# Plachtaa/FAcodec

Hardware: NVIDIA H100
Metric: audio_seconds_per_second (higher is better)
Workload: dtype f32 I/O and accumulation; every product is a 3-MMA split of fp32 operands: fp16 hi + 2^11-scaled fp16 lo (22 mantissa bits, register-promoted accumulation) upstream of the VQ, bf16 hi + bf16 lo (16 bits) downstream

## Files before the change

### facodec_b200/_lib.py

```python
import ctypes
import os

from . import build as _build

_c = ctypes
_LIB = None


class FacError(RuntimeError):
    pass


def lib_path():
    return _build.LIB


def load():
    global _LIB
    if _LIB is not None:
        return _LIB
    path = lib_path()
    if not os.path.exists(path):
        raise FacError(f"{path} not found: build it with `python -m facodec_b200.build` "
                       "(needs nvcc; there is no CPU fallback)")
# ... 37 lines not shown
        "fac_vc_stream_convert": ([vp, i32, i64p, i64p, i32, i32, fp, vp], i32),
        "fac_vc_stream_finish": ([vp, i32, fp, vp], i32),
        "fac_vc_stream_end": ([vp, i32], i32),
        "fac_spectral_loss": ([vp, fp, fp, i32, i32, i32, i32, _c.POINTER(_c.c_int), _c.POINTER(_c.c_int), fp, fp,
                               _c.c_float, _c.c_float, _c.c_float, _c.c_float, fp, vp], i32),
        "fac_l1_loss": ([vp, fp, fp, _c.c_longlong, fp, vp], i32),
        "fac_spectral_loss_grad": ([vp, fp, fp, i32, i32, i32, i32, _c.POINTER(_c.c_int), _c.POINTER(_c.c_int), fp, fp,
                                    _c.c_float, _c.c_float, _c.c_float, _c.c_float, fp, fp, fp, vp], i32),
        "fac_l1_loss_grad": ([vp, fp, fp, _c.c_longlong, fp, fp, fp, vp], i32),
        "fac_add3": ([vp, fp, fp, fp, _c.c_longlong, fp, vp], i32),
        "fac_reconstruction_loss": ([vp, fp, fp, i32, i32, fp, fp, vp], i32),
        "fac_rvq_forward": ([vp, i32, fp, i32, i32, i32, fp, i64p, fp, vp], i32),
        "fac_alias_free_act": ([vp, fp, i32, i32, i32, i32, fp, fp, fp, vp], i32),
        "fac_debug_conv": ([vp, fp, fp, fp] + [i32] * 10 + [fp, fp, i32, fp, fp, i32, vp], i32),
        "fac_debug_conv_tc": ([vp, fp, fp, fp] + [i32] * 10 + [fp, fp, i32, fp, fp, i32, i32, vp], i32),
        "fac_debug_resunit": ([vp, fp, fp, fp, fp, fp, fp, fp, i32, i32, i32, i32, i32, fp, vp], i32),
        "fac_debug_tc_phase_clocks": ([vp, _c.POINTER(_c.c_longlong)], i32),
        "fac_debug_tc_producer_clocks": ([vp, _c.POINTER(_c.c_longlong)], i32),
        "fac_debug_tc_trace": ([vp, _c.POINTER(_c.c_longlong)], i32),
        "fac_debug_lstm_pack": ([fp, i32, i32, fp, _c.c_longlong, _c.POINTER(_c.c_int)], _c.c_longlong),
        "fac_debug_convtr_pack": ([fp, i32, i32, i32, i32, fp, _c.c_longlong], _c.c_longlong),
        "fac_debug_pad_map": ([i32, i32, i32, i32, _c.POINTER(_c.c_int), i32], i32),
        "fac_debug_tc_plan": ([i32] * 8 + [_c.POINTER(_c.c_int)], i32),
        "fac_debug_tc_pack": ([fp, i32, i32, i32, i32, i32, fp, _c.c_longlong], _c.c_longlong),
        "fac_debug_lstm_phase_clocks": ([vp, _c.POINTER(_c.c_longlong)], i32),
        "fac_set_option": ([vp, _c.c_char_p, i32], i32),
        "fac_debug_slstm": ([vp, fp, _c.POINTER(vp), i32, i32, i32, i32, _c.POINTER(_c.c_int), i32, fp, vp], i32),
        "fac_debug_fa_quantize": ([vp, fp, fp, _c.POINTER(vp), fp, i32, i32, i32, i32, i32, fp, fp, fp, fp, i64p, i64p, i64p,
                                   fp, fp, vp], i32),
        "fac_debug_attention": ([vp, fp, fp, fp, fp, i32, i32, i32, _c.c_void_p, i32, vp], i32),
        "fac_debug_tap": ([vp, _c.c_char_p, fp, _c.c_size_t], i32),
        "fac_profile_enable": ([vp, i32], i32),
        "fac_profile_reset": ([vp], i32),
        "fac_profile_get": ([vp, _c.c_char_p, _c.POINTER(_c.c_double), _c.POINTER(_c.c_double),
                             _c.POINTER(_c.c_double), _c.POINTER(_c.c_longlong)], i32),
        "fac_profile_dump": ([vp, _c.c_char_p, _c.c_size_t], _c.c_size_t),
        "fac_workspace_bytes": ([vp], _c.c_size_t),
        "fac_last_launch_count": ([vp], i32),
    }
    for name, (args, res) in sigs.items():
        fn = getattr(L, name)
        fn.argtypes = args
        fn.restype = res
    _LIB = L
    return L


EXPORTED = ["fac_abi_version", "fac_create", "fac_destroy", "fac_last_error", "fac_load_tensor", "fac_finalize",
            "fac_encode", "fac_encode_frames", "fac_quantize", "fac_decode", "fac_codec_forward",
            "fac_codec_forward_host", "fac_codec_encode", "fac_dequantize", "fac_codes_decode", "fac_redecode", "fac_redecoder_decode", "fac_voice_convert", "fac_dataset_mel", "fac_reconstruction_loss", "fac_spectral_loss", "fac_l1_loss", "fac_spectral_loss_grad", "fac_l1_loss_grad", "fac_head_begin", "fac_head_tensor", "fac_head_finalize", "fac_head_forward", "fac_add3", "fac_stream_begin", "fac_stream_encode", "fac_stream_decode", "fac_stream_decode_codes", "fac_stream_encode_codes", "fac_stream_finish_codes", "fac_stream_end", "fac_vc_stream_lookahead", "fac_vc_stream_begin", "fac_vc_stream_convert", "fac_vc_stream_finish", "fac_vc_stream_end", "fac_rvq_create", "fac_rvq_destroy", "fac_rvq_forward", "fac_alias_free_act",
            "fac_debug_conv", "fac_debug_conv_tc", "fac_debug_resunit", "fac_debug_tc_phase_clocks", "fac_debug_tc_producer_clocks", "fac_debug_tc_trace", "fac_debug_lstm_pack", "fac_debug_convtr_pack", "fac_debug_pad_map", "fac_debug_tc_plan", "fac_debug_tc_pack", "fac_debug_lstm_phase_clocks", "fac_set_option", "fac_debug_slstm", "fac_debug_fa_quantize", "fac_debug_attention", "fac_debug_tap", "fac_profile_enable", "fac_profile_reset", "fac_profile_get", "fac_profile_dump",
            "fac_workspace_bytes", "fac_last_launch_count"]


def check(handle, rc, what):
    if rc < 0:
        msg = load().fac_last_error(handle)
        raise FacError(f"{what} failed (status {rc}): {msg.decode() if msg else ''}")
    return rc
```

### facodec_b200/csrc/conv_tc.cu

```cuda
#include <cuda_bf16.h>
#include <cuda_fp16.h>

#include <cstring>
#include <mutex>

#include "common.cuh"
#include "conv_tc_common.cuh"
#include "kernels.h"

namespace fac {

namespace {

using namespace tc;

enum Prec { P_TF32 = 0, P_BF16 = 1, P_F16S = 2, P_F16X2 = 3, P_NONE = -1 };

template <int P> struct PrecT {
    static constexpr int KG = P == P_TF32 ? 4 : 2;
    static constexpr int planes = P == P_F16S ? 1 : 2;
    static constexpr int ksteps = P == P_TF32 ? 2 : 1;
    static constexpr int kind = P == P_TF32 ? WG_TF32 : (P == P_BF16 ? WG_BF16 : WG_F16);
};

// ... 32 lines not shown
            const int row = tl.row0 + 16 * tl.warp + (tl.lane >> 2) + 8 * h;
            const int col = tl.col0 + 8 * j + 2 * (tl.lane & 3);
            f(row, col, acc[4 * j + 2 * h], acc[4 * j + 2 * h + 1]);
        }
    }
}

template <bool FAST>
__device__ __forceinline__ float act_out(int act, float v, float al, float ia) {
    if (act == ACT_SNAKE) return FAST ? fmaf(ia, sin2_mufu(al * v), v) : snake_fast(v, al, ia);
    if (act == ACT_TANH) return tanhf(v);
    if (act == ACT_MISH) return mish_f(v);
    return v;
}

template <int P1, int P2, bool PROMO, int NI, int MINB = 1, bool TT = false>
__global__ void __launch_bounds__(kThreads, MINB) conv_tc_kernel(TcConvParams p) {
    constexpr bool FUSED = P2 != P_NONE;
    static_assert(!TT || (NI == 64 && !FUSED), "transposed tiles: <= 64 channels x 64 time steps per warpgroup");
    static_assert(NI % 16 == 0 && NI <= (PROMO || MINB == 2 ? 64 : (P1 == P_F16S ? 256 : 128)),
                  "accumulator registers: <= 64 / 128 columns (256 in the one-pass fp16 class at one CTA per SM)");
    constexpr bool F16X2 = P1 == P_F16X2;
    constexpr bool DEC = P1 == P_BF16 || P1 == P_F16S;
    using T1 = PrecT<P1>;
    extern __shared__ __align__(1024) uint8_t smem[];
    uint64_t* full = reinterpret_cast<uint64_t*>(smem);

    const int tid = threadIdx.x, wg = tid >> 7;
    const int BM = 64 * p.MT;
    const int N = p.N, NW = p.MT == 2 ? N : N / 2;
    Tile tl;
    tl.row0 = p.MT == 2 ? 64 * wg : 0;
    tl.col0 = p.MT == 2 ? 0 : wg * NW;
    tl.nw = NW;
    tl.warp = (tid >> 5) & 3;
    tl.lane = tid & 31;
    const int t0 = blockIdx.x * BM, ntile = blockIdx.y, b = blockIdx.z;
    const int Kr = p.Kr, dil = p.dil, Rpad = p.Rpad, nchunk = p.nchunk, S = p.stagesB;
    const int R = BM + (Kr - 1) * dil;
    const uint32_t a_plane = (uint32_t)T1::KG * Rpad * 16, a_bytes = a_plane * T1::planes;
    uint8_t* abuf = smem + kSmemHdr;
    float4* master = reinterpret_cast<float4*>(abuf + 2 * (size_t)a_bytes);
    uint8_t* wbuf = abuf + 2 * (size_t)a_bytes + master_bytes(PROMO, nchunk, p.promote_every, NI);
    uint8_t* a2buf = wbuf + (size_t)S * p.b_slot;
    const uint32_t w_unit1 = (uint32_t)Kr * T1::planes * T1::KG * N * 16;
    const uint32_t w_unit2 = FUSED ? (uint32_t)prec_planes(P2) * prec_kg(P2) * N * 16 : 0;
    const int units = nchunk + (FUSED ? p.nchunk2 : 0);

    if (tid == 0) {
        for (int i = 0; i < S; ++i) mbar_init(&full[i], 1);
        fence_mbar_init();
    }
    __syncthreads();
    auto issue_w = [&](int u) {
        uint64_t* bar = &full[u % S];
        uint8_t* dst = wbuf + (size_t)(u % S) * p.b_slot;
        const uint8_t* src;
        uint32_t bytes;
        if (u < nchunk) { src = reinterpret_cast<const uint8_t*>(p.wblob) + ((size_t)ntile * nchunk + u) * w_unit1; bytes = w_unit1; }
        else { src = reinterpret_cast<const uint8_t*>(p.wblob2) + (size_t)(u - nchunk) * w_unit2; bytes = w_unit2; }
        mbar_arrive_expect_tx(bar, bytes);
        bulk_g2s(dst, src, bytes, bar);
    };
    if (tid == 0)
        for (int u = 0; u < S - 1 && u < units; ++u) issue_w(u);

    const PadMap pm = PadMap::make(p.Tin, p.pad_left_s, p.pad_right_s, p.reflect);
    const float* __restrict__ xb = p.x + (size_t)b * p.x_bstride;
    auto produce = [&](int c) {
        uint8_t* ahi = abuf + (size_t)(c & 1) * a_bytes;
        if constexpr (P1 == P_TF32) produce_chunk<kThreads, false>(p, pm, xb, c, t0, R, Rpad, ahi, ahi + a_plane, tid);
        else if constexpr (P1 == P_BF16) produce_chunk<kThreads, true>(p, pm, xb, c, t0, R, Rpad, ahi, ahi + a_plane, tid);
        else if constexpr (P1 == P_F16S) produce_chunk<kThreads, true, 4, false, false, true>(p, pm, xb, c, t0, R, Rpad, ahi, ahi, tid);
        else produce_chunk<kThreads, false, 4, false, true>(p, pm, xb, c, t0, R, Rpad, ahi, ahi + a_plane, tid);
        fence_proxy_async();
    };
    produce(0);

    float acc[NI / 2];
    float crs[F16X2 ? NI / 2 : 1];
    zero_acc<NI>(acc);
    if constexpr (F16X2) zero_acc<NI>(crs);
    const uint32_t a_lbo = (uint32_t)Rpad * 16, b_lbo = (uint32_t)N * 16;
    const uint32_t abase = smem_u32(abuf), wbase = smem_u32(wbuf), a2base = smem_u32(a2buf);
    const int BM2 = BM;

    auto promote = [&](bool first, bool last) {
        if constexpr (PROMO) {
#pragma unroll
// ... 11 lines not shown
                acc[4 * q + 0] = last ? m.x : 0.f;
                acc[4 * q + 1] = last ? m.y : 0.f;
                acc[4 * q + 2] = last ? m.z : 0.f;
                acc[4 * q + 3] = last ? m.w : 0.f;
            }
        }
    };

#pragma unroll 1
    for (int u = 0; u < units; ++u) {
        __syncthreads();
        if (tid == 0 && u + S - 1 < units) issue_w(u + S - 1);
        mbar_wait(&full[u % S], (uint32_t)(u / S) & 1u);
        const uint32_t wslot = wbase + (uint32_t)(u % S) * p.b_slot;
        wg_fence();
        if (u < nchunk) {
            const uint32_t a0 = abase + (uint32_t)(u & 1) * a_bytes + (uint32_t)tl.row0 * 16;
            const uint32_t b0 = wslot + (uint32_t)tl.col0 * 16;
#pragma unroll 1
            for (int tap = 0; tap < Kr; ++tap) {
                const uint32_t ahi = a0 + (uint32_t)(tap * dil) * 16, alo = ahi + a_plane;
                const uint32_t bhi = b0 + (uint32_t)tap * T1::planes * T1::KG * b_lbo, blo = bhi + T1::KG * b_lbo;
                if constexpr (TT) {
                    mma_pass<P1, NI>(acc, bhi, b_lbo, ahi, a_lbo);
                    mma_pass<P1, NI>(crs, bhi, b_lbo, alo, a_lbo);
                    mma_pass<P1, NI>(crs, blo, b_lbo, ahi, a_lbo);
                } else if constexpr (P1 == P_F16S) {
                    mma_pass<P1, NI>(acc, ahi, a_lbo, bhi, b_lbo);
                } else if constexpr (F16X2) {
                    mma_pass<P1, NI>(acc, ahi, a_lbo, bhi, b_lbo);
                    mma_pass<P1, NI>(crs, ahi, a_lbo, blo, b_lbo);
                    mma_pass<P1, NI>(crs, alo, a_lbo, bhi, b_lbo);
                } else {
                    mma_pass<P1, NI>(acc, ahi, a_lbo, bhi, b_lbo);
                    mma_pass<P1, NI>(acc, ahi, a_lbo, blo, b_lbo);
                    mma_pass<P1, NI>(acc, alo, a_lbo, bhi, b_lbo);
                }
            }
            wg_commit();
            if (u + 1 < nchunk) produce(u + 1);
            wg_wait_all();
            if (PROMO && ((u + 1) % p.promote_every == 0 || u + 1 == nchunk)) promote(u < p.promote_every, u + 1 == nchunk);
            if constexpr (FUSED) {
                if (u + 1 == nchunk) {
                    constexpr int KG2 = prec_kg(P2 < 0 ? 0 : P2);
                    const uint32_t a2_plane = (uint32_t)(p.nchunk2 * KG2) * BM2 * 16;
                    for_each_pair<NI, 32>(tl, acc, [&](int row, int col, float v0, float v1) {
                        const float2 bi = __ldg(reinterpret_cast<const float2*>(p.bias + col));
                        const float2 al = __ldg(reinterpret_cast<const float2*>(p.out_alpha + col));
                        const float2 ia = __ldg(reinterpret_cast<const float2*>(p.out_inv_alpha + col));
                        v0 = act_out<DEC>(ACT_SNAKE, v0 + bi.x, al.x, ia.x);
                        v1 = act_out<DEC>(ACT_SNAKE, v1 + bi.y, al.y, ia.y);
                        if constexpr (P2 == P_BF16) {
                            __nv_bfloat162 h = __floats2bfloat162_rn(v0, v1);
                            float2 hf = __bfloat1622float2(h);
                            __nv_bfloat162 l = __floats2bfloat162_rn(v0 - hf.x, v1 - hf.y);
                            const uint32_t off = ((uint32_t)(col >> 3) * BM2 + row) * 16 + (col & 7) * 2;
                            *reinterpret_cast<__nv_bfloat162*>(a2buf + off) = h;
                            *reinterpret_cast<__nv_bfloat162*>(a2buf + a2_plane + off) = l;
                        } else {
                            const float h0 = to_tf32(v0), h1 = to_tf32(v1);
                            const uint32_t off = ((uint32_t)(col >> 2) * BM2 + row) * 16 + (col & 3) * 4;
                            *reinterpret_cast<float2*>(a2buf + off) = make_float2(h0, h1);
                            *reinterpret_cast<float2*>(a2buf + a2_plane + off) = make_float2(to_tf32(v0 - h0), to_tf32(v1 - h1));
                        }
                    });
                    fence_proxy_async();
                    zero_acc<NI>(acc);
                }
            }
        } else if constexpr (FUSED) {
            constexpr int P2x = P2 < 0 ? 0 : P2;
            constexpr int KG2 = prec_kg(P2x);
            const int c2 = u - nchunk;
            const uint32_t a2_plane = (uint32_t)(p.nchunk2 * KG2) * BM2 * 16, a2_lbo = (uint32_t)BM2 * 16;
            const uint32_t ahi = a2base + ((uint32_t)(c2 * KG2) * BM2 + tl.row0) * 16, alo = ahi + a2_plane;
            const uint32_t bhi = wslot + (uint32_t)tl.col0 * 16, blo = bhi + KG2 * b_lbo;
            mma_pass<P2x, NI>(acc, ahi, a2_lbo, bhi, b_lbo);
            mma_pass<P2x, NI>(acc, ahi, a2_lbo, blo, b_lbo);
            mma_pass<P2x, NI>(acc, alo, a2_lbo, bhi, b_lbo);
            wg_commit();
            wg_wait_all();
        }
    }

    const float* __restrict__ bias = FUSED ? p.bias2 : p.bias;
    const int act = FUSED ? ACT_NONE : p.out_act;
    float* __restrict__ yb = p.y + (size_t)b * p.y_bstride + (size_t)ntile * N;
    const float* __restrict__ rb = p.res ? p.res + (size_t)b * p.y_bstride + (size_t)ntile * N : nullptr;
// ... 59 lines not shown
    p.nchunk2 = p.fused ? p.Cout / kChunk : 0;
    p.promote_every = p.promoted ? (p.f16x2 ? (48 / p.Kr < 1 ? 1 : 48 / p.Kr) : (8 / p.Kr < 1 ? 1 : 8 / p.Kr)) : 1;
    const int nw_max = p.promoted ? 64 : 128;
    constexpr size_t kAReserve = 40 * 1024;
    int N = 0;
    for (int cand = p.fused ? p.Cout : 256; cand >= 16 && N == 0; cand -= 16) {
        const bool rows_split = cand <= nw_max, cols_split = (cand / 2) % 16 == 0 && cand / 2 <= nw_max;
        if (p.Cout % cand || !(rows_split || cols_split)) continue;
        size_t slot = (size_t)p.Kr * prec_planes(P1) * prec_kg(P1) * cand * 16, a2 = 0;
        if (P2 != P_NONE) a2 = (size_t)prec_planes(P2) * p.nchunk2 * prec_kg(P2) * 64 * 16;
        if (kSmemHdr + kAReserve + slot + a2 <= kSmemCap) N = cand;
        else if (p.fused) return false;
    }
    if (N == 0) return false;
    struct Layout { int Rpad; size_t slot, total; };
    auto layout = [&](int S, int MT) {
        const int NW = MT == 2 ? N : N / 2, BM = 64 * MT;
        Layout l;
        l.Rpad = BM + (p.Kr - 1) * p.dil;
        while (l.Rpad % 8 != 2) ++l.Rpad;
        const size_t a_bytes = (size_t)prec_planes(P1) * prec_kg(P1) * l.Rpad * 16;
        l.slot = (size_t)p.Kr * prec_planes(P1) * prec_kg(P1) * N * 16;
        size_t a2 = 0;
        if (P2 != P_NONE) {
            const size_t slot2 = (size_t)prec_planes(P2) * prec_kg(P2) * N * 16;
            if (slot2 > l.slot) l.slot = slot2;
            a2 = (size_t)prec_planes(P2) * p.nchunk2 * prec_kg(P2) * BM * 16;
        }
        const size_t master = master_bytes(p.promoted, p.nchunk, p.promote_every, p.tt ? 64 : NW);
        l.total = kSmemHdr + 2 * a_bytes + master + S * l.slot + a2 + (p.tt ? 64 * 16 : 0);
        return l;
    };
    const bool want2 = p.promoted ? !p.tt : (p.occ2_maxn > 0 && N <= p.occ2_maxn);
    for (int two = want2 ? 1 : 0; two >= 0; --two) {
        const size_t cap = two ? kSmemCap2 : kSmemCap;
        const int nwl = two ? 64 : nw_max;
        for (int S = 2; S >= 1; --S)
            for (int MT = 2; MT >= 1; --MT) {
                const int NW = MT == 2 ? N : N / 2;
                const bool wide = !two && P1 == P_F16S && NW == f16s_wide_nw(p.fused);
                if ((NW > nwl && !wide) || NW % 16) continue;
                if (wide && layout(2, 1).total <= kSmemCap2) continue;
                const Layout l = layout(S, MT);
                if (l.total > cap) continue;
                p.N = N; p.MT = MT; p.Rpad = l.Rpad; p.R2pad = 64 * MT; p.stagesB = S; p.b_slot = (int)l.slot;
                p.smem_bytes = l.total;
                p.occ2 = two;
                return true;
            }
    }
    return false;
}

size_t tc_blob_floats(const TcConvParams& p) {
    if (p.g1f16) return (size_t)(p.Cout / p.N) * p.nchunk * p.Kr * 2 * p.N * 4;
    return (size_t)(p.Cout / p.N) * p.nchunk * p.Kr * 2 * ((p.bf16 || p.f16x2) ? 2 : 4) * p.N * 4;
}

static inline uint16_t bf16_rn_host(float f) {
    uint32_t u;
// ... 149 lines not shown
```

### facodec_b200/csrc/conv_tc_common.cuh

```cuda
#pragma once
#include <cuda_bf16.h>
#include <cuda_fp16.h>

#include "common.cuh"
#include "kernels.h"

namespace fac {

namespace tc {

constexpr int kThreads = 256;
constexpr int kChunk = 16;
constexpr int kSmemHdr = 128;

__device__ __forceinline__ uint32_t smem_u32(const void* p) { return (uint32_t)__cvta_generic_to_shared(p); }

__device__ __forceinline__ void mbar_init(uint64_t* bar, uint32_t count) {
    asm volatile("mbarrier.init.shared::cta.b64 [%0], %1;" ::"r"(smem_u32(bar)), "r"(count));
}
__device__ __forceinline__ void mbar_arrive(uint64_t* bar) {
    asm volatile("mbarrier.arrive.shared::cta.b64 _, [%0];" ::"r"(smem_u32(bar)) : "memory");
}
__device__ __forceinline__ void mbar_arrive_expect_tx(uint64_t* bar, uint32_t bytes) {
    asm volatile("mbarrier.arrive.expect_tx.shared::cta.b64 _, [%0], %1;" ::"r"(smem_u32(bar)), "r"(bytes) : "memory");
// ... 194 lines not shown
    uint2 hv, lv;
    hv.x = *reinterpret_cast<uint32_t*>(&h01); hv.y = *reinterpret_cast<uint32_t*>(&h23);
    lv.x = *reinterpret_cast<uint32_t*>(&l01); lv.y = *reinterpret_cast<uint32_t*>(&l23);
    *reinterpret_cast<uint2*>(ahi + off) = hv;
    *reinterpret_cast<uint2*>(alo + off) = lv;
}

__device__ __forceinline__ void store_f16_single(float4 x4, int pc, int row, int Rpad, uint8_t* ahi) {
    __half2 h01 = __floats2half2_rn(x4.x, x4.y), h23 = __floats2half2_rn(x4.z, x4.w);
    const size_t off = ((size_t)(pc >> 1) * Rpad + row) * 16 + (size_t)(pc & 1) * 8;
    uint2 hv;
    hv.x = *reinterpret_cast<uint32_t*>(&h01); hv.y = *reinterpret_cast<uint32_t*>(&h23);
    *reinterpret_cast<uint2*>(ahi + off) = hv;
}

template <int NT, bool BF16, int BATCH = 4, bool INL = false, bool F16 = false, bool SINGLE = false>
__device__ __forceinline__ void produce_chunk(const TcConvParams& p, const PadMap& pm, const float* __restrict__ xb,
                                              int c, int t0, int R, int Rpad, uint8_t* ahi, uint8_t* alo, int ptid) {
    const int pc = ptid & 3;
    const int j = c * kChunk + pc * 4;
    const int soff = j / p.Cin, ci = j - soff * p.Cin;
    const bool has_alpha = p.in_alpha != nullptr;
    float4 al = make_float4(0.f, 0.f, 0.f, 0.f), ia = al;
    if (has_alpha) {
        al = __ldg(reinterpret_cast<const float4*>(p.in_alpha + ci));
        ia = __ldg(reinterpret_cast<const float4*>(p.in_inv_alpha + ci));
    }
    constexpr int RSTEP = NT / 4;
    const int row_limit = p.Tout + (p.Kr - 1) * p.dil;
    const int vrow0 = t0 - p.PLr;
    const float* __restrict__ xcol = xb + ci;
#pragma unroll 1
    for (int r = ptid >> 2; r < R; r += RSTEP * BATCH) {
        float4 v[BATCH];
#pragma unroll
        for (int u = 0; u < BATCH; ++u) {
            const int rr = r + u * RSTEP;
            v[u] = make_float4(0.f, 0.f, 0.f, 0.f);
            const int vrow = vrow0 + rr;
            if (rr < R && vrow < row_limit) {
                const int src = pm.src(vrow * p.vf + soff);
                if (src >= 0) v[u] = __ldg(reinterpret_cast<const float4*>(xcol + (size_t)src * p.ldx));
            }
        }
#pragma unroll
        for (int u = 0; u < BATCH; ++u) {
            const int rr = r + u * RSTEP;
            if (rr < R) {
// ... 14 lines not shown
```

### facodec_b200/csrc/engine.cu

```cuda
#include <cmath>
#include <cstdio>
#include <cstdlib>
#include <cstring>
#include <map>
#include <string>
#include <vector>

#include "../../include/facodec_b200.h"
#include "../../include/facodec_b200_debug.h"
#include "common.cuh"
#include "kernels.h"

using namespace fac;

namespace {

constexpr int HOP = 300;
constexpr int LATENT = 1024;
constexpr int N_FFT = 2048;
constexpr int WIN = 1200;
constexpr int N_BINS = 1025;
constexpr int SPEC_LD = 2052;
constexpr int SPEC_TC_LD = 2176;
constexpr int N_MELS = 80;
// ... 2713 lines not shown
    if (std::string(name) == "fuse_resunit") { h->fuse_res = value < 0 ? 0 : (value > 2 ? 2 : value); return FAC_OK; }
    if (std::string(name) == "encoder_f16x2") { h->enc_f16 = value != 0; return FAC_OK; }
    if (std::string(name) == "encoder_tt") { h->enc_tt = value != 0; return FAC_OK; }
    if (std::string(name) == "tc_occ2_maxn") { h->tc_occ2 = value < 0 ? 0 : value; return FAC_OK; }
    if (std::string(name) == "decoder_conv7_fp16") { h->dec_c7_f16 = value != 0; return FAC_OK; }
    if (std::string(name) == "overlap_front") { h->overlap_front = value != 0; return FAC_OK; }
    if (std::string(name) == "lstm_v2") { h->lstm_v2 = value != 0; return FAC_OK; }
    if (std::string(name) == "decoder_lstm_fp16") { h->dec_lstm_fp16 = value != 0; return FAC_OK; }
    if (std::string(name) == "attention_stream") { h->attn_stream = value != 0; return FAC_OK; }
    if (std::string(name) == "decoder_bf16") { h->dec_bf16 = value != 0; return FAC_OK; }
    if (std::string(name) == "tensor_cores") { h->use_tc = value < 0 ? 0 : (value > 2 ? 2 : value); return FAC_OK; }
    h->err = std::string("unknown option ") + name;
    return FAC_ERR_INVALID;
}

int fac_debug_conv_tc(fac_handle* h, const float* x, const float* w_host, const float* bias_host, int B, int Tin, int Cin,
                      int Cout, int K, int dil, int stride, int pad_left, int pad_right, int reflect,
                      const float* in_alpha_host, const float* out_alpha_host, int act, const float* res, float* y,
                      int Tout, int promoted, void* stream) {
    if (!h || !x || !w_host || !y) return FAC_ERR_INVALID;
    cudaSetDevice(h->device);
    cudaStream_t st = (cudaStream_t)stream;
    TcConvParams tp;
    tp.Cin = Cin; tp.Cout = Cout; tp.promoted = (promoted == 1 || promoted == 3 || promoted == 4) ? 1 : 0;
    tp.bf16 = (promoted == 2 || promoted == 5) ? 1 : 0;
    tp.f16x2 = (promoted == 3 || promoted == 4) ? 1 : 0;
    tp.tt = promoted == 4 ? 1 : 0;
    tp.g1f16 = promoted == 5 ? 1 : 0;
    tp.occ2_maxn = h->tc_occ2;
    tp.Tout = Tout;
    if (stride == 1) { tp.vf = 1; tp.Kr = K; tp.dil = dil; }
    else if (K == 2 * stride && dil == 1) { tp.vf = stride; tp.Kr = 2; tp.dil = 1; }
    else { h->err = "fac_debug_conv_tc: unsupported stride/kernel"; return FAC_ERR_UNSUPPORTED; }
    if (promoted < 0 || promoted > 5 || !tc_conv_plan(tp)) { h->err = "fac_debug_conv_tc: layer not eligible for the tensor-core path"; return FAC_ERR_UNSUPPORTED; }
    int ldw = (Cout + 3) / 4 * 4;
    std::vector<float> gen((size_t)K * Cin * ldw, 0.f);
    for (int co = 0; co < Cout; ++co)
        for (int ci = 0; ci < Cin; ++ci)
            for (int k = 0; k < K; ++k) gen[((size_t)k * Cin + ci) * ldw + co] = w_host[((size_t)co * Cin + ci) * K + k];
    size_t nb = tc_blob_floats(tp);
    auto al4 = [](size_t v) { return (v + 3) / 4 * 4; };
    size_t o_b = al4(nb), o_ia = al4(o_b + Cout), o_iia = al4(o_ia + Cin), o_oa = al4(o_iia + Cin), o_oia = al4(o_oa + Cout);
    std::vector<float> pk(o_oia + Cout + 16, 0.f);
    tc_pack_blob(tp, gen.data(), ldw, pk.data());
    for (int i = 0; i < Cout; ++i) pk[o_b + i] = bias_host ? bias_host[i] : 0.f;
    for (int i = 0; i < Cin; ++i) { pk[o_ia + i] = in_alpha_host ? in_alpha_host[i] : 1.f; pk[o_iia + i] = 1.0f / (pk[o_ia + i] + 1e-9f); }
    for (int i = 0; i < Cout; ++i) { pk[o_oa + i] = out_alpha_host ? out_alpha_host[i] : 1.f; pk[o_oia + i] = 1.0f / (pk[o_oa + i] + 1e-9f); }
    float* d = nullptr;
    cudaError_t e = cudaMalloc(&d, pk.size() * sizeof(float));
// ... 2 lines not shown
    tp.x = x; tp.y = y; tp.wblob = d; tp.bias = d + o_b;
    if (in_alpha_host) { tp.in_alpha = d + o_ia; tp.in_inv_alpha = d + o_iia; }
    tp.out_act = act;
    if (out_alpha_host) { tp.out_act = ACT_SNAKE; tp.out_alpha = d + o_oa; tp.out_inv_alpha = d + o_oia; }
    tp.res = res;
    tp.B = B; tp.Tin = Tin; tp.ldx = Cin;
    tp.PLr = pad_left / tp.vf;
    tp.pad_left_s = pad_left; tp.pad_right_s = pad_right; tp.reflect = reflect;
    tp.Tout = Tout; tp.ldy = Cout;
    tp.x_bstride = (size_t)Tin * Cin; tp.y_bstride = (size_t)Tout * Cout;
    e = launch_conv_tc(tp, st);
    if (e == cudaSuccess) e = cudaStreamSynchronize(st);
    cudaFree(d);
    if (e != cudaSuccess) { h->err = std::string("fac_debug_conv_tc: ") + cudaGetErrorString(e); return FAC_ERR_CUDA; }
    return FAC_OK;
}

int fac_debug_resunit(fac_handle* h, const float* x, const float* w7_host, const float* b7_host, const float* w1_host,
                      const float* b1_host, const float* alpha1_host, const float* alpha2_host, int B, int T, int C,
                      int dil, int mode, float* y, void* stream) {
    if (!h || !x || !y || !w7_host || !w1_host) return FAC_ERR_INVALID;
    fac_handle tmp;
    tmp.device = h->device;
    tmp.use_tc = mode == 0 ? 0 : 1;
    tmp.fuse_res = (mode == 2 || mode == 4 || mode == 6) ? 1 : 0;
    tmp.dec_bf16 = mode >= 3;
    tmp.dec_c7_f16 = mode >= 5;
    tmp.tc_occ2 = h->tc_occ2;
    auto put = [&](const char* key, const float* d, std::vector<int64_t> shp) {
        HostTensor t;
// ... 77 lines not shown
    const long long n = (long long)c.K * Cin * c.Cout;
    if (!out || capacity_floats < n) return n;
    for (int k = 0; k < c.K; ++k)
        for (int ci = 0; ci < Cin; ++ci)
            for (int co = 0; co < c.Cout; ++co) out[((size_t)k * Cin + ci) * c.Cout + co] = tmp.pack[c.w + ((size_t)k * Cin + ci) * c.ldw + co];
    return n;
}

int fac_debug_pad_map(int L, int pad_left, int pad_right, int reflect, int* out, int n) {
    if (!out || L < 0 || pad_left < 0 || pad_right < 0 || n != pad_left + L + pad_right) return FAC_ERR_INVALID;
    const PadMap pm = PadMap::make(L, pad_left, pad_right, reflect);
    for (int i = 0; i < n; ++i) out[i] = pm.src(i - pad_left);
    return FAC_OK;
}

int fac_debug_tc_plan(int Cin, int Cout, int K, int dil, int stride, int Tout, int mode, int occ2_maxn, int* out8) {
    if (!out8 || Cin <= 0 || Cout <= 0 || K <= 0 || dil <= 0 || stride <= 0 || mode < 0 || mode > 8) return FAC_ERR_INVALID;
    TcConvParams tp;
    tp.Cin = Cin; tp.Cout = Cout; tp.Tout = Tout; tp.occ2_maxn = occ2_maxn;
    tp.promoted = (mode == 1 || mode == 3) ? 1 : 0;
    tp.bf16 = (mode == 2 || mode == 4 || mode == 7 || mode == 8) ? 1 : 0;
    tp.f16x2 = mode == 3 ? 1 : 0;
    tp.fused = (mode == 4 || mode == 5 || mode == 8) ? 1 : 0;
    tp.g1f16 = (mode == 7 || mode == 8) ? 1 : 0;
    if (mode == 6) { tp.promoted = 1; tp.f16x2 = 1; tp.tt = 1; }
    if (stride == 1) { tp.vf = 1; tp.Kr = K; tp.dil = dil; }
    else if (K == 2 * stride && dil == 1) { tp.vf = stride; tp.Kr = 2; tp.dil = 1; }
    else return FAC_ERR_UNSUPPORTED;
    if (!tc_conv_plan(tp)) return FAC_ERR_UNSUPPORTED;
    out8[0] = tp.N; out8[1] = tp.MT; out8[2] = tp.nchunk; out8[3] = tp.stagesB; out8[4] = tp.R2pad;
    out8[5] = (int)tp.smem_bytes; out8[6] = tp.Rpad; out8[7] = tp.promote_every;
    return FAC_OK;
}

long long fac_debug_tc_pack(const float* w_host, int Cin, int Cout, int K, int stride, int mode, float* blob_out,
                            long long capacity_floats) {
    if (!w_host || Cin <= 0 || Cout <= 0 || K <= 0 || stride <= 0 || mode < 0 || mode > 3) return FAC_ERR_INVALID;
    TcConvParams tp;
    tp.Cin = Cin; tp.Cout = Cout; tp.dil = 1;
    tp.promoted = (mode == 1 || mode == 3) ? 1 : 0; tp.bf16 = mode == 2 ? 1 : 0; tp.f16x2 = mode == 3 ? 1 : 0;
    if (stride == 1) { tp.vf = 1; tp.Kr = K; }
    else if (K == 2 * stride) { tp.vf = stride; tp.Kr = 2; }
    else return FAC_ERR_UNSUPPORTED;
    if (!tc_conv_plan(tp)) return FAC_ERR_UNSUPPORTED;
    const long long n = (long long)tc_blob_floats(tp);
    if (!blob_out || capacity_floats < n) return n;
    const int ldw = (Cout + 3) / 4 * 4;
// ... 109 lines not shown
```

### facodec_b200/csrc/kernels.h

```cpp
#pragma once
#include <cuda_runtime.h>
#include <stdint.h>

namespace fac {

struct ConvParams {
    const float* x = nullptr;
    const float* w = nullptr;
    const float* bias = nullptr;
    const float* in_alpha = nullptr;
    const float* in_inv_alpha = nullptr;
    const float* out_alpha = nullptr;
    const float* out_inv_alpha = nullptr;
    const float* res = nullptr;
    const int* valid_len = nullptr;
    float* y = nullptr;
    int B = 0, Tin = 0, Cin = 0, Tout = 0, Cout = 0;
    int K = 1, dil = 1, stride = 1, pad_left = 0, pad_right = 0, pad_reflect = 0;
    int ldw = 0, ldy = 0, ldx = 0;
    int out_act = 0;
    int y_transposed = 0;
    size_t x_bstride = 0, y_bstride = 0;
};
cudaError_t launch_conv(const ConvParams& p, cudaStream_t st);
// ... 9 lines not shown
    const float* res = nullptr;
    float* y = nullptr;
    int B = 0, Tin = 0, Cin = 0, ldx = 0;
    int vf = 1;
    int Kr = 1, dil = 1, PLr = 0;
    int pad_left_s = 0, pad_right_s = 0, reflect = 0;
    int Tout = 0, Cout = 0, ldy = 0;
    int out_act = 0;
    int promoted = 0;
    int bf16 = 0;
    int g1f16 = 0;
    int f16x2 = 0;
    int fused = 0;
    int tt = 0;
    int occ2_maxn = 0;
    const float* wblob2 = nullptr;
    const float* bias2 = nullptr;
    int nchunk2 = 0;
    int promote_every = 1;
    int N = 0, nchunk = 0, Rpad = 0, stagesB = 0;
    int MT = 2;
    int b_slot = 0;
    int occ2 = 0;
    int R2pad = 0;
    size_t smem_bytes = 0;
    size_t x_bstride = 0, y_bstride = 0;
};
bool tc_conv_plan(TcConvParams& p);
size_t tc_blob_floats(const TcConvParams& p);
void tc_pack_blob(const TcConvParams& p, const float* wp, int ldw, float* blob);
cudaError_t launch_conv_tc(const TcConvParams& p, cudaStream_t st);

struct LstmParams {
    const float* xg = nullptr;
    const float* whh_p = nullptr;
// ... 108 lines not shown
```

### include/facodec_b200_debug.h

```cpp
#ifndef FACODEC_B200_DEBUG_H
#define FACODEC_B200_DEBUG_H

#include "facodec_b200.h"

#ifdef __cplusplus
extern "C" {
#endif

int fac_debug_conv(fac_handle* h, const float* x, const float* w_host, const float* bias_host, int B, int Tin,
                   int Cin, int Cout, int K, int dil, int stride, int pad_left, int pad_right, int reflect,
                   const float* in_alpha_host, const float* out_alpha_host, int act, const float* res,
                   float* y, int Tout, void* stream);
int fac_debug_conv_tc(fac_handle* h, const float* x, const float* w_host, const float* bias_host, int B, int Tin,
                      int Cin, int Cout, int K, int dil, int stride, int pad_left, int pad_right, int reflect,
                      const float* in_alpha_host, const float* out_alpha_host, int act, const float* res,
                      float* y, int Tout, int promoted, void* stream);
int fac_debug_resunit(fac_handle* h, const float* x, const float* w7_host, const float* b7_host, const float* w1_host,
                      const float* b1_host, const float* alpha1_host, const float* alpha2_host, int B, int T, int C,
                      int dil, int mode, float* y, void* stream);
int fac_debug_tc_phase_clocks(fac_handle* h, long long* out8);
int fac_debug_tc_producer_clocks(fac_handle* h, long long* out4);
int fac_debug_tc_trace(fac_handle* h, long long* out80);
long long fac_debug_lstm_pack(const float* whh_host, int H, int bf16, float* out, long long capacity_floats, int* info3);
int fac_debug_pad_map(int L, int pad_left, int pad_right, int reflect, int* out, int n);
int fac_debug_tc_plan(int Cin, int Cout, int K, int dil, int stride, int Tout, int mode, int occ2_maxn, int* out8);
long long fac_debug_tc_pack(const float* w_host, int Cin, int Cout, int K, int stride, int mode, float* blob_out,
                            long long capacity_floats);
int fac_debug_lstm_phase_clocks(fac_handle* h, long long* out4);
long long fac_debug_convtr_pack(const float* w_host, int Cin, int Cout, int stride, int causal, float* out,
                                long long capacity_floats);
int fac_debug_slstm(fac_handle* h, const float* x, const float* const* w_host, int B, int T, int H, int upstream,
                    const int* chunks, int n_chunks, float* y, void* stream);
int fac_debug_fa_quantize(fac_handle* h, const float* f0, const float* z, const float* const vq_host[6][5],
                          const float* gamma_beta, int n_c, int B, int Tq, int Tz, int Tf0, float* outs, float* zp,
                          float* zc, float* zr, int64_t* codes_p, int64_t* codes_c, int64_t* codes_r, float* sqerr,
                          float* losses2, void* stream);
int fac_debug_attention(fac_handle* h, const float* q, const float* k, const float* v, float* o, int B, int T,
                        int heads, const int* valid_len, int force_stream, void* stream);
int fac_debug_tap(fac_handle* h, const char* name, float* dst, size_t capacity_floats);

// ... 11 lines not shown
```

Before: 920.6.

## Group multiple input-channel chunks per pipeline step in tensor-core conv

The tensor-core conv kernel can now process G (2 or 4) input-channel chunks per pipeline stage. Each stage loads a G-times larger weight slot with one bulk copy and runs G*Kr MMA taps between waits, which cuts the number of barrier, commit and wait round trips and the producer iterations. The producer spreads threads across more channel columns, the A-buffer row padding changes with G, and launch bounds request two CTAs per SM for groupable variants. In exchange it uses more shared memory, which can reduce occupancy, and the higher min-blocks bound may force register spills. Debug entry points are added to compare against a forced G=1 plan.

```diff
diff --git a/facodec_b200/_lib.py b/facodec_b200/_lib.py
--- a/facodec_b200/_lib.py
+++ b/facodec_b200/_lib.py
@@ -75,6 +75,8 @@
         "fac_alias_free_act": ([vp, fp, i32, i32, i32, i32, fp, fp, fp, vp], i32),
         "fac_debug_conv": ([vp, fp, fp, fp] + [i32] * 10 + [fp, fp, i32, fp, fp, i32, vp], i32),
         "fac_debug_conv_tc": ([vp, fp, fp, fp] + [i32] * 10 + [fp, fp, i32, fp, fp, i32, i32, vp], i32),
+        "fac_debug_conv_tc_group1": ([vp, fp, fp, fp] + [i32] * 10 + [fp, fp, i32, fp, fp, i32, i32, vp,
+                                     _c.POINTER(_c.c_int)], i32),
         "fac_debug_resunit": ([vp, fp, fp, fp, fp, fp, fp, fp, i32, i32, i32, i32, i32, fp, vp], i32),
         "fac_debug_tc_phase_clocks": ([vp, _c.POINTER(_c.c_longlong)], i32),
         "fac_debug_tc_producer_clocks": ([vp, _c.POINTER(_c.c_longlong)], i32),
@@ -83,6 +85,7 @@
         "fac_debug_convtr_pack": ([fp, i32, i32, i32, i32, fp, _c.c_longlong], _c.c_longlong),
         "fac_debug_pad_map": ([i32, i32, i32, i32, _c.POINTER(_c.c_int), i32], i32),
         "fac_debug_tc_plan": ([i32] * 8 + [_c.POINTER(_c.c_int)], i32),
+        "fac_debug_tc_plan_group": ([i32] * 8 + [_c.POINTER(_c.c_int)], i32),
         "fac_debug_tc_pack": ([fp, i32, i32, i32, i32, i32, fp, _c.c_longlong], _c.c_longlong),
         "fac_debug_lstm_phase_clocks": ([vp, _c.POINTER(_c.c_longlong)], i32),
         "fac_set_option": ([vp, _c.c_char_p, i32], i32),
@@ -110,7 +113,7 @@
 EXPORTED = ["fac_abi_version", "fac_create", "fac_destroy", "fac_last_error", "fac_load_tensor", "fac_finalize",
             "fac_encode", "fac_encode_frames", "fac_quantize", "fac_decode", "fac_codec_forward",
             "fac_codec_forward_host", "fac_codec_encode", "fac_dequantize", "fac_codes_decode", "fac_redecode", "fac_redecoder_decode", "fac_voice_convert", "fac_dataset_mel", "fac_reconstruction_loss", "fac_spectral_loss", "fac_l1_loss", "fac_spectral_loss_grad", "fac_l1_loss_grad", "fac_head_begin", "fac_head_tensor", "fac_head_finalize", "fac_head_forward", "fac_add3", "fac_stream_begin", "fac_stream_encode", "fac_stream_decode", "fac_stream_decode_codes", "fac_stream_encode_codes", "fac_stream_finish_codes", "fac_stream_end", "fac_vc_stream_lookahead", "fac_vc_stream_begin", "fac_vc_stream_convert", "fac_vc_stream_finish", "fac_vc_stream_end", "fac_rvq_create", "fac_rvq_destroy", "fac_rvq_forward", "fac_alias_free_act",
-            "fac_debug_conv", "fac_debug_conv_tc", "fac_debug_resunit", "fac_debug_tc_phase_clocks", "fac_debug_tc_producer_clocks", "fac_debug_tc_trace", "fac_debug_lstm_pack", "fac_debug_convtr_pack", "fac_debug_pad_map", "fac_debug_tc_plan", "fac_debug_tc_pack", "fac_debug_lstm_phase_clocks", "fac_set_option", "fac_debug_slstm", "fac_debug_fa_quantize", "fac_debug_attention", "fac_debug_tap", "fac_profile_enable", "fac_profile_reset", "fac_profile_get", "fac_profile_dump",
+            "fac_debug_conv", "fac_debug_conv_tc", "fac_debug_conv_tc_group1", "fac_debug_resunit", "fac_debug_tc_phase_clocks", "fac_debug_tc_producer_clocks", "fac_debug_tc_trace", "fac_debug_lstm_pack", "fac_debug_convtr_pack", "fac_debug_pad_map", "fac_debug_tc_plan", "fac_debug_tc_plan_group", "fac_debug_tc_pack", "fac_debug_lstm_phase_clocks", "fac_set_option", "fac_debug_slstm", "fac_debug_fa_quantize", "fac_debug_attention", "fac_debug_tap", "fac_profile_enable", "fac_profile_reset", "fac_profile_get", "fac_profile_dump",
             "fac_workspace_bytes", "fac_last_launch_count"]
 
 
diff --git a/facodec_b200/csrc/conv_tc.cu b/facodec_b200/csrc/conv_tc.cu
--- a/facodec_b200/csrc/conv_tc.cu
+++ b/facodec_b200/csrc/conv_tc.cu
@@ -3,6 +3,7 @@
 
 #include <cstring>
 #include <mutex>
+#include <type_traits>
 
 #include "common.cuh"
 #include "conv_tc_common.cuh"
@@ -70,9 +71,13 @@
     return v;
 }
 
+template <int P1, int P2, bool TT>
+constexpr bool groupable() { return P1 != P_F16S && P2 == P_NONE && !TT; }
+
 template <int P1, int P2, bool PROMO, int NI, int MINB = 1, bool TT = false>
-__global__ void __launch_bounds__(kThreads, MINB) conv_tc_kernel(TcConvParams p) {
+__global__ void __launch_bounds__(kThreads, groupable<P1, P2, TT>() && NI <= 128 ? 2 : MINB) conv_tc_kernel(TcConvParams p) {
     constexpr bool FUSED = P2 != P_NONE;
+    constexpr bool GROUPABLE = groupable<P1, P2, TT>();
     static_assert(!TT || (NI == 64 && !FUSED), "transposed tiles: <= 64 channels x 64 time steps per warpgroup");
     static_assert(NI % 16 == 0 && NI <= (PROMO || MINB == 2 ? 64 : (P1 == P_F16S ? 256 : 128)),
                   "accumulator registers: <= 64 / 128 columns (256 in the one-pass fp16 class at one CTA per SM)");
@@ -93,15 +98,17 @@
     tl.lane = tid & 31;
     const int t0 = blockIdx.x * BM, ntile = blockIdx.y, b = blockIdx.z;
     const int Kr = p.Kr, dil = p.dil, Rpad = p.Rpad, nchunk = p.nchunk, S = p.stagesB;
+    const int G = GROUPABLE ? p.group : 1;
     const int R = BM + (Kr - 1) * dil;
-    const uint32_t a_plane = (uint32_t)T1::KG * Rpad * 16, a_bytes = a_plane * T1::planes;
+    const int nstep1 = G == 4 ? nchunk >> 2 : (G == 2 ? nchunk >> 1 : nchunk);
+    const uint32_t a_plane = (uint32_t)G * T1::KG * Rpad * 16, a_bytes = a_plane * T1::planes;
     uint8_t* abuf = smem + kSmemHdr;
     float4* master = reinterpret_cast<float4*>(abuf + 2 * (size_t)a_bytes);
     uint8_t* wbuf = abuf + 2 * (size_t)a_bytes + master_bytes(PROMO, nchunk, p.promote_every, NI);
     uint8_t* a2buf = wbuf + (size_t)S * p.b_slot;
     const uint32_t w_unit1 = (uint32_t)Kr * T1::planes * T1::KG * N * 16;
     const uint32_t w_unit2 = FUSED ? (uint32_t)prec_planes(P2) * prec_kg(P2) * N * 16 : 0;
-    const int units = nchunk + (FUSED ? p.nchunk2 : 0);
+    const int units = nstep1 + (FUSED ? p.nchunk2 : 0);
 
     if (tid == 0) {
         for (int i = 0; i < S; ++i) mbar_init(&full[i], 1);
@@ -113,8 +120,10 @@
         uint8_t* dst = wbuf + (size_t)(u % S) * p.b_slot;
         const uint8_t* src;
         uint32_t bytes;
-        if (u < nchunk) { src = reinterpret_cast<const uint8_t*>(p.wblob) + ((size_t)ntile * nchunk + u) * w_unit1; bytes = w_unit1; }
-        else { src = reinterpret_cast<const uint8_t*>(p.wblob2) + (size_t)(u - nchunk) * w_unit2; bytes = w_unit2; }
+        if (u < nstep1) {
+            src = reinterpret_cast<const uint8_t*>(p.wblob) + ((size_t)ntile * nchunk + (size_t)u * G) * w_unit1;
+            bytes = G * w_unit1;
+        } else { src = reinterpret_cast<const uint8_t*>(p.wblob2) + (size_t)(u - nstep1) * w_unit2; bytes = w_unit2; }
         mbar_arrive_expect_tx(bar, bytes);
         bulk_g2s(dst, src, bytes, bar);
     };
@@ -123,12 +132,22 @@
 
     const PadMap pm = PadMap::make(p.Tin, p.pad_left_s, p.pad_right_s, p.reflect);
     const float* __restrict__ xb = p.x + (size_t)b * p.x_bstride;
-    auto produce = [&](int c) {
-        uint8_t* ahi = abuf + (size_t)(c & 1) * a_bytes;
-        if constexpr (P1 == P_TF32) produce_chunk<kThreads, false>(p, pm, xb, c, t0, R, Rpad, ahi, ahi + a_plane, tid);
-        else if constexpr (P1 == P_BF16) produce_chunk<kThreads, true>(p, pm, xb, c, t0, R, Rpad, ahi, ahi + a_plane, tid);
-        else if constexpr (P1 == P_F16S) produce_chunk<kThreads, true, 4, false, false, true>(p, pm, xb, c, t0, R, Rpad, ahi, ahi, tid);
-        else produce_chunk<kThreads, false, 4, false, true>(p, pm, xb, c, t0, R, Rpad, ahi, ahi + a_plane, tid);
+    auto produce = [&](int s) {
+        uint8_t* ahi = abuf + (size_t)(s & 1) * a_bytes;
+        auto run = [&](auto grouped) {
+            constexpr bool GR = decltype(grouped)::value;
+            const int c = GR ? s * G : s;
+            if constexpr (P1 == P_TF32) produce_chunk<kThreads, GR, false>(p, pm, xb, c, G, t0, R, Rpad, ahi, ahi + a_plane, tid);
+            else if constexpr (P1 == P_BF16) produce_chunk<kThreads, GR, true>(p, pm, xb, c, G, t0, R, Rpad, ahi, ahi + a_plane, tid);
+            else if constexpr (P1 == P_F16S) produce_chunk<kThreads, GR, true, 4, false, false, true>(p, pm, xb, c, G, t0, R, Rpad, ahi, ahi, tid);
+            else produce_chunk<kThreads, GR, false, 4, false, true>(p, pm, xb, c, G, t0, R, Rpad, ahi, ahi + a_plane, tid);
+        };
+        if constexpr (GROUPABLE) {
+            if (G > 1) run(std::true_type());
+            else run(std::false_type());
+        } else {
+            run(std::false_type());
+        }
         fence_proxy_async();
     };
     produce(0);
@@ -170,13 +189,11 @@
         mbar_wait(&full[u % S], (uint32_t)(u / S) & 1u);
         const uint32_t wslot = wbase + (uint32_t)(u % S) * p.b_slot;
         wg_fence();
-        if (u < nchunk) {
+        if (u < nstep1) {
             const uint32_t a0 = abase + (uint32_t)(u & 1) * a_bytes + (uint32_t)tl.row0 * 16;
             const uint32_t b0 = wslot + (uint32_t)tl.col0 * 16;
-#pragma unroll 1
-            for (int tap = 0; tap < Kr; ++tap) {
-                const uint32_t ahi = a0 + (uint32_t)(tap * dil) * 16, alo = ahi + a_plane;
-                const uint32_t bhi = b0 + (uint32_t)tap * T1::planes * T1::KG * b_lbo, blo = bhi + T1::KG * b_lbo;
+            auto mma_tap = [&](uint32_t ahi, uint32_t bhi) {
+                const uint32_t alo = ahi + a_plane, blo = bhi + T1::KG * b_lbo;
                 if constexpr (TT) {
                     mma_pass<P1, NI>(acc, bhi, b_lbo, ahi, a_lbo);
                     mma_pass<P1, NI>(crs, bhi, b_lbo, alo, a_lbo);
@@ -192,13 +209,27 @@
                     mma_pass<P1, NI>(acc, ahi, a_lbo, blo, b_lbo);
                     mma_pass<P1, NI>(acc, alo, a_lbo, bhi, b_lbo);
                 }
+            };
+            if constexpr (GROUPABLE) {
+                uint32_t ac = a0, bc = b0, ahi = a0, bhi = b0;
+#pragma unroll 1
+                for (int i = 0, tap = 0; i < G * Kr; ++i) {
+                    mma_tap(ahi, bhi);
+                    if (++tap < Kr) { ahi += (uint32_t)dil * 16; bhi += T1::planes * T1::KG * b_lbo; }
+                    else { tap = 0; ac += T1::KG * a_lbo; bc += w_unit1; ahi = ac; bhi = bc; }
+                }
+            } else {
+#pragma unroll 1
+                for (int tap = 0; tap < Kr; ++tap)
+                    mma_tap(a0 + (uint32_t)(tap * dil) * 16, b0 + (uint32_t)tap * T1::planes * T1::KG * b_lbo);
             }
             wg_commit();
-            if (u + 1 < nchunk) produce(u + 1);
+            if (u + 1 < nstep1) produce(u + 1);
             wg_wait_all();
-            if (PROMO && ((u + 1) % p.promote_every == 0 || u + 1 == nchunk)) promote(u < p.promote_every, u + 1 == nchunk);
+            const int done = (u + 1) * G;
+            if (PROMO && (done % p.promote_every == 0 || done == nchunk)) promote(done <= p.promote_every, done == nchunk);
             if constexpr (FUSED) {
-                if (u + 1 == nchunk) {
+                if (u + 1 == nstep1) {
                     constexpr int KG2 = prec_kg(P2 < 0 ? 0 : P2);
                     const uint32_t a2_plane = (uint32_t)(p.nchunk2 * KG2) * BM2 * 16;
                     for_each_pair<NI, 32>(tl, acc, [&](int row, int col, float v0, float v1) {
@@ -228,7 +259,7 @@
         } else if constexpr (FUSED) {
             constexpr int P2x = P2 < 0 ? 0 : P2;
             constexpr int KG2 = prec_kg(P2x);
-            const int c2 = u - nchunk;
+            const int c2 = u - nstep1;
             const uint32_t a2_plane = (uint32_t)(p.nchunk2 * KG2) * BM2 * 16, a2_lbo = (uint32_t)BM2 * 16;
             const uint32_t ahi = a2base + ((uint32_t)(c2 * KG2) * BM2 + tl.row0) * 16, alo = ahi + a2_plane;
             const uint32_t bhi = wslot + (uint32_t)tl.col0 * 16, blo = bhi + KG2 * b_lbo;
@@ -318,13 +349,14 @@
     }
     if (N == 0) return false;
     struct Layout { int Rpad; size_t slot, total; };
-    auto layout = [&](int S, int MT) {
+    auto layout = [&](int S, int MT, int G) {
         const int NW = MT == 2 ? N : N / 2, BM = 64 * MT;
         Layout l;
+        const int v = G == 1 ? 2 : (P1 == P_TF32 ? 1 : 4 / G);
         l.Rpad = BM + (p.Kr - 1) * p.dil;
-        while (l.Rpad % 8 != 2) ++l.Rpad;
-        const size_t a_bytes = (size_t)prec_planes(P1) * prec_kg(P1) * l.Rpad * 16;
-        l.slot = (size_t)p.Kr * prec_planes(P1) * prec_kg(P1) * N * 16;
+        while (l.Rpad % 8 != v) ++l.Rpad;
+        const size_t a_bytes = (size_t)G * prec_planes(P1) * prec_kg(P1) * l.Rpad * 16;
+        l.slot = (size_t)G * p.Kr * prec_planes(P1) * prec_kg(P1) * N * 16;
         size_t a2 = 0;
         if (P2 != P_NONE) {
             const size_t slot2 = (size_t)prec_planes(P2) * prec_kg(P2) * N * 16;
@@ -334,6 +366,12 @@
         const size_t master = master_bytes(p.promoted, p.nchunk, p.promote_every, p.tt ? 64 : NW);
         l.total = kSmemHdr + 2 * a_bytes + master + S * l.slot + a2 + (p.tt ? 64 * 16 : 0);
         return l;
+    };
+    auto group = [&](int S, int MT, size_t cap) {
+        if (p.Kr > 3 || p.tt || p.fused || p.g1f16) return 1;
+        for (int G = 4; G > 1; G /= 2)
+            if (G <= p.max_group && p.nchunk % G == 0 && (!p.promoted || p.promote_every % G == 0) && layout(S, MT, G).total <= cap) return G;
+        return 1;
     };
     const bool want2 = p.promoted ? !p.tt : (p.occ2_maxn > 0 && N <= p.occ2_maxn);
     for (int two = want2 ? 1 : 0; two >= 0; --two) {
@@ -344,10 +382,13 @@
                 const int NW = MT == 2 ? N : N / 2;
                 const bool wide = !two && P1 == P_F16S && NW == f16s_wide_nw(p.fused);
                 if ((NW > nwl && !wide) || NW % 16) continue;
-                if (wide && layout(2, 1).total <= kSmemCap2) continue;
-                const Layout l = layout(S, MT);
-                if (l.total > cap) continue;
+                if (wide && layout(2, 1, 1).total <= kSmemCap2) continue;
+                const Layout l1 = layout(S, MT, 1);
+                if (l1.total > cap) continue;
+                const int G = group(S, MT, l1.total <= kSmemCap2 ? kSmemCap2 : cap);
+                const Layout l = layout(S, MT, G);
                 p.N = N; p.MT = MT; p.Rpad = l.Rpad; p.R2pad = 64 * MT; p.stagesB = S; p.b_slot = (int)l.slot;
+                p.group = G;
                 p.smem_bytes = l.total;
                 p.occ2 = two;
                 return true;
diff --git a/facodec_b200/csrc/conv_tc_common.cuh b/facodec_b200/csrc/conv_tc_common.cuh
--- a/facodec_b200/csrc/conv_tc_common.cuh
+++ b/facodec_b200/csrc/conv_tc_common.cuh
@@ -232,10 +232,11 @@
     *reinterpret_cast<uint2*>(ahi + off) = hv;
 }
 
-template <int NT, bool BF16, int BATCH = 4, bool INL = false, bool F16 = false, bool SINGLE = false>
+template <int NT, bool GROUPED, bool BF16, int BATCH = 4, bool INL = false, bool F16 = false, bool SINGLE = false>
 __device__ __forceinline__ void produce_chunk(const TcConvParams& p, const PadMap& pm, const float* __restrict__ xb,
-                                              int c, int t0, int R, int Rpad, uint8_t* ahi, uint8_t* alo, int ptid) {
-    const int pc = ptid & 3;
+                                              int c, int G, int t0, int R, int Rpad, uint8_t* ahi, uint8_t* alo, int ptid) {
+    const int lp = GROUPED ? (G == 4 ? 4 : 3) : 2;
+    const int pc = ptid & ((1 << lp) - 1);
     const int j = c * kChunk + pc * 4;
     const int soff = j / p.Cin, ci = j - soff * p.Cin;
     const bool has_alpha = p.in_alpha != nullptr;
@@ -244,12 +245,12 @@
         al = __ldg(reinterpret_cast<const float4*>(p.in_alpha + ci));
         ia = __ldg(reinterpret_cast<const float4*>(p.in_inv_alpha + ci));
     }
-    constexpr int RSTEP = NT / 4;
+    const int RSTEP = NT >> lp;
     const int row_limit = p.Tout + (p.Kr - 1) * p.dil;
     const int vrow0 = t0 - p.PLr;
     const float* __restrict__ xcol = xb + ci;
 #pragma unroll 1
-    for (int r = ptid >> 2; r < R; r += RSTEP * BATCH) {
+    for (int r = ptid >> lp; r < R; r += RSTEP * BATCH) {
         float4 v[BATCH];
 #pragma unroll
         for (int u = 0; u < BATCH; ++u) {
diff --git a/facodec_b200/csrc/engine.cu b/facodec_b200/csrc/engine.cu
--- a/facodec_b200/csrc/engine.cu
+++ b/facodec_b200/csrc/engine.cu
@@ -2751,10 +2751,10 @@
     return FAC_ERR_INVALID;
 }
 
-int fac_debug_conv_tc(fac_handle* h, const float* x, const float* w_host, const float* bias_host, int B, int Tin, int Cin,
-                      int Cout, int K, int dil, int stride, int pad_left, int pad_right, int reflect,
-                      const float* in_alpha_host, const float* out_alpha_host, int act, const float* res, float* y,
-                      int Tout, int promoted, void* stream) {
+static int debug_conv_tc(fac_handle* h, const float* x, const float* w_host, const float* bias_host, int B, int Tin, int Cin,
+                         int Cout, int K, int dil, int stride, int pad_left, int pad_right, int reflect,
+                         const float* in_alpha_host, const float* out_alpha_host, int act, const float* res, float* y,
+                         int Tout, int promoted, void* stream, int* group_out) {
     if (!h || !x || !w_host || !y) return FAC_ERR_INVALID;
     cudaSetDevice(h->device);
     cudaStream_t st = (cudaStream_t)stream;
@@ -2770,6 +2770,11 @@
     else if (K == 2 * stride && dil == 1) { tp.vf = stride; tp.Kr = 2; tp.dil = 1; }
     else { h->err = "fac_debug_conv_tc: unsupported stride/kernel"; return FAC_ERR_UNSUPPORTED; }
     if (promoted < 0 || promoted > 5 || !tc_conv_plan(tp)) { h->err = "fac_debug_conv_tc: layer not eligible for the tensor-core path"; return FAC_ERR_UNSUPPORTED; }
+    if (group_out) {
+        *group_out = tp.group;
+        tp.max_group = 1;
+        if (!tc_conv_plan(tp)) { h->err = "fac_debug_conv_tc_group1: no one-chunk plan"; return FAC_ERR_UNSUPPORTED; }
+    }
     int ldw = (Cout + 3) / 4 * 4;
     std::vector<float> gen((size_t)K * Cin * ldw, 0.f);
     for (int co = 0; co < Cout; ++co)
@@ -2802,6 +2807,23 @@
     cudaFree(d);
     if (e != cudaSuccess) { h->err = std::string("fac_debug_conv_tc: ") + cudaGetErrorString(e); return FAC_ERR_CUDA; }
     return FAC_OK;
+}
+
+int fac_debug_conv_tc(fac_handle* h, const float* x, const float* w_host, const float* bias_host, int B, int Tin, int Cin,
+                      int Cout, int K, int dil, int stride, int pad_left, int pad_right, int reflect,
+                      const float* in_alpha_host, const float* out_alpha_host, int act, const float* res, float* y,
+                      int Tout, int promoted, void* stream) {
+    return debug_conv_tc(h, x, w_host, bias_host, B, Tin, Cin, Cout, K, dil, stride, pad_left, pad_right, reflect,
+                         in_alpha_host, out_alpha_host, act, res, y, Tout, promoted, stream, nullptr);
+}
+
+int fac_debug_conv_tc_group1(fac_handle* h, const float* x, const float* w_host, const float* bias_host, int B, int Tin,
+                             int Cin, int Cout, int K, int dil, int stride, int pad_left, int pad_right, int reflect,
+                             const float* in_alpha_host, const float* out_alpha_host, int act, const float* res, float* y,
+                             int Tout, int promoted, void* stream, int* group) {
+    if (!group) return FAC_ERR_INVALID;
+    return debug_conv_tc(h, x, w_host, bias_host, B, Tin, Cin, Cout, K, dil, stride, pad_left, pad_right, reflect,
+                         in_alpha_host, out_alpha_host, act, res, y, Tout, promoted, stream, group);
 }
 
 int fac_debug_resunit(fac_handle* h, const float* x, const float* w7_host, const float* b7_host, const float* w1_host,
@@ -2909,9 +2931,8 @@
     return FAC_OK;
 }
 
-int fac_debug_tc_plan(int Cin, int Cout, int K, int dil, int stride, int Tout, int mode, int occ2_maxn, int* out8) {
-    if (!out8 || Cin <= 0 || Cout <= 0 || K <= 0 || dil <= 0 || stride <= 0 || mode < 0 || mode > 8) return FAC_ERR_INVALID;
-    TcConvParams tp;
+static int debug_tc_plan(int Cin, int Cout, int K, int dil, int stride, int Tout, int mode, int occ2_maxn, TcConvParams& tp) {
+    if (Cin <= 0 || Cout <= 0 || K <= 0 || dil <= 0 || stride <= 0 || mode < 0 || mode > 8) return FAC_ERR_INVALID;
     tp.Cin = Cin; tp.Cout = Cout; tp.Tout = Tout; tp.occ2_maxn = occ2_maxn;
     tp.promoted = (mode == 1 || mode == 3) ? 1 : 0;
     tp.bf16 = (mode == 2 || mode == 4 || mode == 7 || mode == 8) ? 1 : 0;
@@ -2922,10 +2943,31 @@
     if (stride == 1) { tp.vf = 1; tp.Kr = K; tp.dil = dil; }
     else if (K == 2 * stride && dil == 1) { tp.vf = stride; tp.Kr = 2; tp.dil = 1; }
     else return FAC_ERR_UNSUPPORTED;
-    if (!tc_conv_plan(tp)) return FAC_ERR_UNSUPPORTED;
+    return tc_conv_plan(tp) ? FAC_OK : FAC_ERR_UNSUPPORTED;
+}
+
+int fac_debug_tc_plan(int Cin, int Cout, int K, int dil, int stride, int Tout, int mode, int occ2_maxn, int* out8) {
+    if (!out8) return FAC_ERR_INVALID;
+    TcConvParams tp;
+    const int rc = debug_tc_plan(Cin, Cout, K, dil, stride, Tout, mode, occ2_maxn, tp);
+    if (rc != FAC_OK) return rc;
     out8[0] = tp.N; out8[1] = tp.MT; out8[2] = tp.nchunk; out8[3] = tp.stagesB; out8[4] = tp.R2pad;
     out8[5] = (int)tp.smem_bytes; out8[6] = tp.Rpad; out8[7] = tp.promote_every;
     return FAC_OK;
+}
+
+int fac_debug_tc_plan_group(int Cin, int Cout, int K, int dil, int stride, int Tout, int mode, int occ2_maxn, int* smem2) {
+    TcConvParams tp;
+    const int rc = debug_tc_plan(Cin, Cout, K, dil, stride, Tout, mode, occ2_maxn, tp);
+    if (rc != FAC_OK) return rc;
+    if (smem2) {
+        TcConvParams t1 = tp;
+        t1.max_group = 1;
+        if (!tc_conv_plan(t1)) return FAC_ERR_UNSUPPORTED;
+        smem2[0] = (int)tp.smem_bytes;
+        smem2[1] = (int)t1.smem_bytes;
+    }
+    return tp.group;
 }
 
 long long fac_debug_tc_pack(const float* w_host, int Cin, int Cout, int K, int stride, int mode, float* blob_out,
diff --git a/facodec_b200/csrc/kernels.h b/facodec_b200/csrc/kernels.h
--- a/facodec_b200/csrc/kernels.h
+++ b/facodec_b200/csrc/kernels.h
@@ -47,11 +47,13 @@
     int fused = 0;
     int tt = 0;
     int occ2_maxn = 0;
+    int max_group = 4;
     const float* wblob2 = nullptr;
     const float* bias2 = nullptr;
     int nchunk2 = 0;
     int promote_every = 1;
     int N = 0, nchunk = 0, Rpad = 0, stagesB = 0;
+    int group = 1;
     int MT = 2;
     int b_slot = 0;
     int occ2 = 0;
diff --git a/include/facodec_b200_debug.h b/include/facodec_b200_debug.h
--- a/include/facodec_b200_debug.h
+++ b/include/facodec_b200_debug.h
@@ -15,6 +15,10 @@
                       int Cin, int Cout, int K, int dil, int stride, int pad_left, int pad_right, int reflect,
                       const float* in_alpha_host, const float* out_alpha_host, int act, const float* res,
                       float* y, int Tout, int promoted, void* stream);
+int fac_debug_conv_tc_group1(fac_handle* h, const float* x, const float* w_host, const float* bias_host, int B, int Tin,
+                             int Cin, int Cout, int K, int dil, int stride, int pad_left, int pad_right, int reflect,
+                             const float* in_alpha_host, const float* out_alpha_host, int act, const float* res,
+                             float* y, int Tout, int promoted, void* stream, int* group);
 int fac_debug_resunit(fac_handle* h, const float* x, const float* w7_host, const float* b7_host, const float* w1_host,
                       const float* b1_host, const float* alpha1_host, const float* alpha2_host, int B, int T, int C,
                       int dil, int mode, float* y, void* stream);
@@ -24,6 +28,7 @@
 long long fac_debug_lstm_pack(const float* whh_host, int H, int bf16, float* out, long long capacity_floats, int* info3);
 int fac_debug_pad_map(int L, int pad_left, int pad_right, int reflect, int* out, int n);
 int fac_debug_tc_plan(int Cin, int Cout, int K, int dil, int stride, int Tout, int mode, int occ2_maxn, int* out8);
+int fac_debug_tc_plan_group(int Cin, int Cout, int K, int dil, int stride, int Tout, int mode, int occ2_maxn, int* smem2);
 long long fac_debug_tc_pack(const float* w_host, int Cin, int Cout, int K, int stride, int mode, float* blob_out,
                             long long capacity_floats);
 int fac_debug_lstm_phase_clocks(fac_handle* h, long long* out4);
```

Result: faster. 1004 (median of 6 runs) (+9.0%).
